# storj/uplink

Hardware: AMD Instinct MI355X
Metric: GiB/s erasure encode+decode (device-resident), RS(29,80) 64 MiB segments (higher is better)
Workload: dtype u8

## Files before the change

uplink_amd/csrc/ec_sets.cpp:

```cpp
#include "ec_internal.hpp"

namespace uplink_ec {
namespace capi {
namespace {


struct SetSeg {
    const uint8_t *in[kMaxOps];
    int num[kMaxOps];
    int missing[kMaxOps];
    int nin = 0, nstore = 0, rows = 0, nw = 2;
    uint8_t *out = nullptr;
};

int set_segment(const ec_ctx *c, int nshares, const int *nums, const uint8_t *const *pieces, uint8_t *out,
                bool decode, SetSeg &sg) {
    const int k = c->k;
    std::vector<int> order, ids;
    int rc = choose_shares(c, nshares, nums, order, ids);
    if (rc) return rc;
    if (decode)
        for (int i = 0; i < nshares; i++)
            if (nums[i] < 0 || nums[i] >= c->n) return EC_ERR_INVALID_SHARE;
    bool seen[256] = {};
// ... 32 lines not shown
    SetsSlot *sl = nullptr;
    const auto t_end = std::chrono::steady_clock::now() + std::chrono::milliseconds(SetsRing::kAcquireTimeoutMs);
    for (;;) {
        {
            std::lock_guard<std::mutex> g(R.mu);
            size_t live = 0;
            for (auto &x : R.slots) {
                live += !x->dead;
                if (!sl && x->idle()) sl = x.get();
            }
            if (!sl && live < SetsRing::kMaxSlots) {
                auto x = std::make_unique<SetsSlot>();
                if (hipHostMalloc((void **)&x->h_words, 4 * (SetsRing::kInitSegs + 1), kSetsHostFlags) != hipSuccess)
                    return nullptr;
                memset(x->h_words, 0, 4 * (SetsRing::kInitSegs + 1));
                x->words_cap = SetsRing::kInitSegs + 1;
                x->stage_cap = 0;
                R.slots.push_back(std::move(x));
                sl = R.slots.back().get();
            }
            if (sl) sl->busy = true;
        }
        if (sl) break;
        if (std::chrono::steady_clock::now() > t_end) return nullptr;
        std::this_thread::sleep_for(std::chrono::microseconds(20));
    }
    bool ok = true;
    if (sl->stage_cap < nseg) {
        size_t cap = std::max(sl->stage_cap ? 2 * sl->stage_cap : SetsRing::kInitSegs, (size_t)32);
        while (cap < nseg) cap *= 2;
        if (sl->h_stage) sl->old_host.push_back(sl->h_stage);
        for (void *p : {(void *)sl->d_stage, (void *)sl->d_desc, (void *)sl->d_words})
            if (p) sl->old_dev.push_back(p);
        sl->h_stage = nullptr, sl->d_stage = nullptr, sl->d_desc = nullptr, sl->d_words = nullptr;
        ok = hipHostMalloc((void **)&sl->h_stage, cap * sizeof(SetStage),
                           c->sets_stage_dma ? hipHostMallocDefault : kSetsHostFlags) == hipSuccess &&
             (!c->sets_stage_dma || hipMalloc(&sl->d_stage, cap * sizeof(SetStage)) == hipSuccess) &&
             hipMalloc(&sl->d_desc, cap * sizeof(SetDesc)) == hipSuccess &&
             hipMalloc(&sl->d_words, 4 * (cap + 1)) == hipSuccess;
        if (ok && cap + 1 > sl->words_cap) {
            uint32_t *hw = nullptr;
            ok = hipHostMalloc((void **)&hw, 4 * (cap + 1), kSetsHostFlags) == hipSuccess;
            if (ok) {
                hw[0] = sl->seq;
                sl->old_host.push_back(sl->h_words);
                sl->h_words = hw;
                sl->words_cap = cap + 1;
            }
        }
        sl->stage_cap = ok ? cap : 0;
    }
    if (ok && sl->tgt_cap < tgt_words) {
        size_t cap = std::max(sl->tgt_cap ? 2 * sl->tgt_cap : SetsRing::kInitTgtWords, (size_t)1);
        while (cap < tgt_words) cap *= 2;
        if (sl->d_tgt) sl->old_dev.push_back(sl->d_tgt);
        sl->d_tgt = nullptr;
        ok = hipMalloc(&sl->d_tgt, cap * 8) == hipSuccess;
        sl->tgt_cap = ok ? cap : 0;
    }
    if (!ok) {
        std::lock_guard<std::mutex> g(R.mu);
        sl->busy = false;
        return nullptr;
    }
    return sl;
}

void sets_release(ec_ctx *c, SetsSlot *sl) {
    std::lock_guard<std::mutex> g(c->sets.mu);
    sl->busy = false;
}

int sets_call(ec_ctx *c, std::vector<SetSeg> &segs, int64_t nstripes, hipStream_t s, std::vector<uint32_t> *bad) {
    const int k = c->k, ess = c->ess;
    const size_t nseg = segs.size();
    if (nseg == 0 || nstripes == 0) return EC_OK;
    if (c->sets_merge) {
        int nw = 2;
        for (auto &sg : segs) nw = std::max(nw, sg.nw);
        for (auto &sg : segs) sg.nw = nw;
    }
    {
        const int64_t tiles_seg = (nstripes * (ess / 16) + kTileChunksHost - 1) / kTileChunksHost;
        const int64_t per = share_max_tiles(4) / tiles_seg;
        if (per < 1) return EC_ERR_UNSUPPORTED;
        if ((int64_t)nseg > per) {
            for (size_t g0 = 0; g0 < nseg; g0 += (size_t)per) {
                std::vector<SetSeg> part(segs.begin() + g0, segs.begin() + std::min(nseg, g0 + (size_t)per));
                std::vector<uint32_t> pbad;
                const int rc = sets_call(c, part, nstripes, s, bad ? &pbad : nullptr);
                if (rc) return rc;
                if (bad) bad->insert(bad->end(), pbad.begin(), pbad.end());
            }
            return EC_OK;
        }
    }
    std::vector<int> idx(nseg);
    for (size_t g = 0; g < nseg; g++) idx[g] = (int)g;
    std::stable_sort(idx.begin(), idx.end(), [&](int x, int y) { return segs[x].nw < segs[y].nw; });
    std::vector<size_t> toff(nseg);
    size_t words = 0;
    for (size_t q = 0; q < nseg; q++) {
        toff[q] = words;
        words += (leaf_entries(segs[idx[q]].nin, segs[idx[q]].rows, segs[idx[q]].nw) + 7) & ~(size_t)7;
    }
    if (stream_is_capturing(s)) return EC_ERR_UNSUPPORTED;
    SetsSlot *sl = sets_acquire(c, nseg, words);
    if (!sl) return EC_ERR_DEVICE;
    SetStage one{};
    const bool in_args = nseg == 1 && !sl->d_stage;
    SetStage *stage = in_args ? &one : sl->h_stage;
    for (size_t q = 0; q < nseg; q++) {
        const SetSeg &sg = segs[idx[q]];
        SetStage &st = stage[q];
        SetDesc &d = st.d;
        for (int j = 0; j < sg.nin; j++) {
            d.in[j] = sg.in[j];
            d.copy_off[j] = j < k && sg.num[j] < k ? sg.num[j] * ess : -1;
            st.num[j] = sg.num[j];
        }
        for (int r = 0; r < sg.nstore; r++) {
            d.out_off[r] = sg.missing[r] * ess;
            st.missing[r] = sg.missing[r];
        }
        d.out = sg.out;
        d.tgt = sl->d_tgt + toff[q];
        d.zero_check = bad ? sl->d_words + 1 + q : nullptr;
        d.nin = sg.nin;
        d.nout = sg.rows;
        d.nstore = sg.nstore;
        d.status = 0;
        st.k = k;
        st.nw = sg.nw;
    }
    const uint32_t seq = sl->seq + 1;
    const int64_t chunks = nstripes * (ess / 16), tiles = (chunks + kTileChunksHost - 1) / kTileChunksHost;
    auto pass_args = [&](SetsArgs &a) {
        a.nstripes = nstripes;
        a.chunks_per_seg = chunks;
        a.tiles_per_seg = tiles;
        a.ess = ess;
        a.cps = ess / 16;
        a.k = k;
        a.done_ctr = sl->d_words;
        a.host_done = sl->h_words;
        a.seq = seq;
        a.total_wgs = (uint32_t)(tiles * (int64_t)nseg);
        a.chk_flag = c->d_chk;
        a.jt_base = c->jt_base;
    };
    hipError_t e = hipSuccess;
    if (in_args && !bad && c->sets_one && segs[0].nin <= kOneMaxIn && segs[0].nin * segs[0].rows <= kOneMaxCoef) {
        const SetSeg &sg = segs[0];
        SetOne p{};
        pass_args(p.a);
        p.a.total_tiles = tiles;
        for (int j = 0; j < sg.nin; j++) {
            p.in[j] = one.d.in[j];
            p.copy_off[j] = one.d.copy_off[j];
        }
        for (int r = 0; r < sg.nstore; r++) p.out_off[r] = one.d.out_off[r];
        p.out = sg.out;
        p.tgt = sl->d_tgt;
        p.nin = sg.nin;
        p.nout = sg.rows;
        p.nstore = sg.nstore;
        solve_rows(sg.num, k, sg.nin, sg.missing, sg.nstore, p.coef);
        e = launch_sets_one(p, sg.nw, s);
        if (e != hipSuccess) {
            sets_release(c, sl);
            return hip_fail(e);
        }
        sl->seq = seq;
        c->last_body = EC_BODY_JUMP_TABLE;
        const int rc = after_launch(c->d_chk, s);
        sets_release(c, sl);
        return rc;
    }
    if (sl->d_stage)
        e = hipMemcpyAsync(sl->d_stage, sl->h_stage, nseg * sizeof(SetStage), hipMemcpyHostToDevice, s);
    if (e == hipSuccess)
        e = in_args ? launch_sets_prep1(one, sl->d_desc, c->jt_base, sl->d_words, s)
                    : launch_sets_prep(sl->d_stage ? sl->d_stage : sl->h_stage, sl->d_desc, (int)nseg, c->jt_base,
                                       sl->d_words, s);
    if (e != hipSuccess) {
        sets_release(c, sl);
        return hip_fail(e);
    }
    for (size_t q0 = 0; q0 < nseg && e == hipSuccess;) {
        size_t q1 = q0;
        while (q1 < nseg && segs[idx[q1]].nw == segs[idx[q0]].nw) q1++;
        SetsArgs a{};
        pass_args(a);
        a.desc = sl->d_desc + q0;
        a.total_tiles = tiles * (int64_t)(q1 - q0);
        e = launch_matmul_sets(a, segs[idx[q0]].nw, s);
        q0 = q1;
    }
    if (e != hipSuccess) {
        const bool drained = hipStreamSynchronize(s) == hipSuccess && hipMemset(sl->d_words, 0, 4) == hipSuccess;
        std::lock_guard<std::mutex> g(c->sets.mu);
        sl->dead = !drained;
        sl->busy = false;
        return hip_fail(e);
    }
    sl->seq = seq;
    c->last_body = EC_BODY_JUMP_TABLE;
    int rc = after_launch(c->d_chk, s);
    if (bad && rc == EC_OK) {
        if (hipMemcpyAsync(sl->h_words + 1, sl->d_words + 1, 4 * nseg, hipMemcpyDeviceToHost, s) != hipSuccess ||
            hipStreamSynchronize(s) != hipSuccess)
            rc = EC_ERR_DEVICE;
        bad->assign(nseg, 0);
        for (size_t q = 0; q < nseg && rc == EC_OK; q++) (*bad)[idx[q]] = sl->h_words[1 + q];
    }
    sets_release(c, sl);
    return rc;
}


std::mutex g_builders_mu;
std::set<ec_ctx *> g_builders;

void sl_worker(ec_ctx *c) {
    (void)hipSetDevice(c->device);
    SlBuilder &B = c->slb;
    for (;;) {
        std::vector<int> ids;
        {
            std::unique_lock<std::mutex> g(B.mu);
            B.cv.wait(g, [&] { return B.stop || !B.q.empty(); });
            if (B.stop) break;
            ids = std::move(B.q.front());
            B.q.pop_front();
        }
        PlanPtr plan;
        if (get_plan(c, ids, &plan) == EC_OK && plan->rows >= 1 && plan->rows <= kMaxOps) ensure_sl(c, *plan);
        {
            std::lock_guard<std::mutex> g(B.mu);
            B.pending.erase(ids);
        }
        B.cv.notify_all();
    }
    std::lock_guard<std::mutex> g(B.mu);
    B.pending.clear();
    B.q.clear();
    B.cv.notify_all();
}

void stop_builders() {
    std::lock_guard<std::mutex> g(g_builders_mu);
    for (ec_ctx *c : g_builders) {
        {
            std::lock_guard<std::mutex> b(c->slb.mu);
            c->slb.stop = true;
        }
        c->slb.cv.notify_all();
        if (c->slb.th.joinable()) c->slb.th.join();
    }
    g_builders.clear();
}

void stop_builder_impl(ec_ctx *c) {
    {
        std::lock_guard<std::mutex> g(g_builders_mu);
        g_builders.erase(c);
        {
            std::lock_guard<std::mutex> b(c->slb.mu);
            c->slb.stop = true;
        }
        c->slb.cv.notify_all();
    }
    if (c->slb.th.joinable()) c->slb.th.join();
}

void sl_request(ec_ctx *c, const std::vector<int> &ids) {
    SlBuilder &B = c->slb;
    std::lock_guard<std::mutex> g(B.mu);
// ... 165 lines not shown
```

uplink_amd/csrc/rs_repair.hip:

```cpp
#include <hip/hip_runtime.h>

#include "gf256_field.hpp"
#include "rs_repair.hpp"
#include "rs_sets_tile.hpp"

namespace uplink_ec {
namespace {

using namespace dev;

__constant__ GfTables c_gf = make_gf_tables();

__global__ __launch_bounds__(256) void rs_repair_prep(const RepairStage *stage, RepairDesc *desc, uint64_t jt_base) {
    const RepairStage *st = stage + blockIdx.x;
    copy_desc(&st->d, desc + blockIdx.x);
    write_leaves(st->coef, st->entries, st->d.tgt, jt_base);
}

typedef const __attribute__((address_space(4))) RepairDesc ConstDesc;

struct RepairGeom {
    static constexpr bool kCopy = false, kOwnTable = false;
    const RepairArgs &a;
    ConstDesc *d;
    const int nstore;
    bool vA, vB;
    int64_t iA, iB, oA, oB;
    uint32_t bad = 0;

    __device__ __forceinline__ bool skip(int nin, int nout) const { return nin <= 0 || nout <= 0; }
    __device__ __forceinline__ void cols(int lane) {
        const int64_t tile = blockIdx.x;
        const int64_t seg = tile / a.tiles_per_seg;
        const int64_t qA = (tile - seg * a.tiles_per_seg) * kTileChunks + lane, qB = qA + 64;
        vA = qA < a.chunks_per_seg, vB = qB < a.chunks_per_seg;
        iA = vA ? qA * 16 : 0, iB = vB ? qB * 16 : 0;
        oA = qA * 16, oB = qB * 16;
    }
    __device__ __forceinline__ bool in_ok(const uint8_t *p, const uint8_t *share) const {
        return in_span(a, p, share, a.piece_len, 10);
    }
    __device__ __forceinline__ bool out_ok(const uint8_t *p, const uint8_t *row) const {
        return in_span(a, p, row, a.piece_len, 11);
    }
    __device__ __forceinline__ uint8_t *row_out(int r) const { return d->out[r]; }
    __device__ __forceinline__ int stored(int, int) const { return nstore; }
    __device__ __forceinline__ bool checks(int rbase, int cnt, int nst) const { return rbase + cnt > nst; }
    __device__ __forceinline__ void report(uint32_t any, int) { bad |= any; }
    __device__ __forceinline__ void finish(int lane) const {
        if (d->nout > nstore) {
            int32_t *st = d->status;
            if (__ballot(bad != 0) != 0 && lane == 0 && st) atomicOr(st, 1);
        }
    }
};

template <int NW>
__global__ __launch_bounds__(NW * 64, 4) void rs_repair(const RepairArgs a) {
    ConstDesc *d = (ConstDesc *)(a.desc + blockIdx.x / a.tiles_per_seg);
    RepairGeom G{a, d, d->nstore};
    share_tile<NW>(G);
}


__global__ __launch_bounds__(256) void rs_repair_sized_prep(const RepairSizedStage *stage, RepairSizedDesc *desc,
                                                            uint64_t jt_base) {
    const RepairSizedStage *st = stage + blockIdx.x;
    copy_desc(&st->d, desc + blockIdx.x);
    uint32_t *map = st->map;
    const int64_t ntiles = st->ntiles;
    for (int64_t i = threadIdx.x; i < ntiles; i += blockDim.x) map[i] = blockIdx.x;
    write_leaves(st->coef, st->entries, st->d.tgt, jt_base);
}

typedef const __attribute__((address_space(4))) RepairSizedDesc ConstSizedDesc;
typedef const __attribute__((address_space(4))) uint32_t ConstMap;

struct RepairSizedGeom {
    static constexpr bool kCopy = false, kOwnTable = false;
    const RepairSizedArgs &a;
    ConstSizedDesc *d;
    const int64_t tile;
    const int nstore;
    bool vA, vB;
    int64_t iA, iB, oA, oB;
    uint32_t bad = 0;

    __device__ __forceinline__ RepairSizedGeom(const RepairSizedArgs &a_, int64_t ctile)
        : a(a_),
          d((ConstSizedDesc *)(a_.desc + (uint32_t)__builtin_amdgcn_readfirstlane(((ConstMap *)a_.map)[ctile]))),
          tile(ctile - d->tile0), nstore(d->nstore) {}
    __device__ __forceinline__ bool skip(int nin, int nout) const { return nin <= 0 || nout <= 0 || tile < 0; }
    __device__ __forceinline__ void cols(int lane) {
        const int64_t chunks = d->chunks;
        const int64_t qA = tile * kTileChunks + lane, qB = qA + 64;
        vA = qA < chunks, vB = qB < chunks;
        iA = vA ? qA * 16 : 0, iB = vB ? qB * 16 : 0;
        oA = qA * 16, oB = qB * 16;
    }
    __device__ __forceinline__ bool in_ok(const uint8_t *p, const uint8_t *share) const {
        return in_span(a, p, share, d->piece_len, 14);
    }
    __device__ __forceinline__ bool out_ok(const uint8_t *p, const uint8_t *row) const {
        return in_span(a, p, row, d->piece_len, 15);
    }
    __device__ __forceinline__ uint8_t *row_out(int r) const { return d->out[r]; }
    __device__ __forceinline__ int stored(int, int) const { return nstore; }
    __device__ __forceinline__ bool checks(int rbase, int cnt, int nst) const { return rbase + cnt > nst; }
    __device__ __forceinline__ void report(uint32_t any, int) { bad |= any; }
    __device__ __forceinline__ void finish(int lane) const {
        if (d->nout > nstore) {
            int32_t *st = d->status;
            if (__ballot(bad != 0) != 0 && lane == 0 && st) atomicOr(st, 1);
        }
    }
};

template <int NW>
__global__ __launch_bounds__(NW * 64, 4) void rs_repair_sized(const RepairSizedArgs a) {
    RepairSizedGeom G(a, a.tile_base + blockIdx.x);
    share_tile<NW>(G);
}

__global__ __launch_bounds__(256) void rs_repair_check_bytes(const RsArgs a) {
    __shared__ uint8_t s_exp[512];
    __shared__ uint8_t s_log[256];
    __shared__ int s_bad;
    for (int i = threadIdx.x; i < 512; i += blockDim.x) s_exp[i] = c_gf.exp[i];
    for (int i = threadIdx.x; i < 256; i += blockDim.x) s_log[i] = c_gf.log[i];
    if (threadIdx.x == 0) s_bad = 0;
    __syncthreads();
    const int64_t cols = a.nstripes * a.ess;
    bool bad = false;
    for (int64_t col = (int64_t)blockIdx.x * blockDim.x + threadIdx.x; col < cols; col += (int64_t)gridDim.x * blockDim.x) {
        for (int r = 0; r < a.nout; r++) {
            uint8_t acc = 0;
            for (int j = 0; j < a.nin; j++) {
                const uint8_t x = a.in_base[a.in_off[j] + col];
                const uint8_t cv = a.coef[(int64_t)j * a.coef_ld + r];
                if (x && cv) acc ^= s_exp[s_log[x] + s_log[cv]];
            }
            bad = bad || acc != a.out_base[a.out_off[r] + col];
        }
    }
    if (bad) s_bad = 1;
    __syncthreads();
    if (threadIdx.x == 0 && s_bad) atomicOr(a.zero_check, 1u);
}

}

int repair_waves(int rows) { return rows <= 14 ? 2 : rows <= 24 ? 3 : rows <= 32 ? 4 : 8; }

hipError_t launch_repair_prep(const RepairStage *stage, RepairDesc *desc, int nseg, uint64_t jt_base, hipStream_t s) {
    if (nseg <= 0) return hipSuccess;
    hipLaunchKernelGGL(rs_repair_prep, dim3(nseg), dim3(256), 0, s, stage, desc, jt_base);
    return hipGetLastError();
}

hipError_t launch_repair(const RepairArgs &a, int nw, hipStream_t s) {
    return launch_share_tile(a, a.total_tiles, nw, s, rs_repair<2>, rs_repair<3>, rs_repair<4>, rs_repair<8>);
}
// ... 24 lines not shown
```

uplink_amd/csrc/rs_sets.hip:

```cpp
#include <hip/hip_runtime.h>

#include "../../include/uplink_ec.h"
#include "gf256_field.hpp"
#include "rs_device.hpp"
#include "rs_kernels.hpp"
#include "rs_sets.hpp"
#include "rs_sets_tile.hpp"

namespace uplink_ec {
namespace {

using namespace dev;

__constant__ GfTables c_gf = make_gf_tables();

__device__ __forceinline__ void solve_rows(const SetStage *st, uint64_t jt_base) {
    __shared__ uint8_t s_exp[512], s_log[256];
    __shared__ uint8_t s_x[kMaxOps];
    __shared__ uint8_t s_y[2 * kMaxOps];
    __shared__ int16_t s_lw[kMaxOps];
    __shared__ int16_t s_ln[2 * kMaxOps], s_hit[2 * kMaxOps];
    __shared__ int s_num[kMaxOps], s_miss[kMaxOps];
    __shared__ int s_acc[kMaxOps + 2 * kMaxOps];
    __shared__ int s_hdr[8];
// ... 4 lines not shown
        s_miss[i] = st->missing[i];
    }
    if (tid == 0) s_hdr[0] = st->d.nin;
    if (tid == 1) s_hdr[1] = st->d.nout;
    if (tid == 2) s_hdr[2] = st->d.nstore;
    if (tid == 3) s_hdr[3] = st->nw;
    if (tid == 4) s_hdr[4] = st->k;
    if (tid == 5) s_tgt = st->d.tgt;
    for (int i = tid; i < 512; i += nt) s_exp[i] = c_gf.exp[i];
    for (int i = tid; i < 256; i += nt) s_log[i] = c_gf.log[i];
    __syncthreads();
    const int nin = s_hdr[0], nout = s_hdr[1], nstore = s_hdr[2], nw = s_hdr[3], k = s_hdr[4];
    auto point = [&](int num) -> uint8_t { return num == 0 ? 0 : s_exp[(num - 1) % 255]; };
    for (int i = tid; i < k; i += nt) s_x[i] = point(s_num[i]);
    for (int i = tid; i < nout; i += nt) s_y[i] = point(i < nstore ? s_miss[i] : s_num[k + i - nstore]);
    for (int i = tid; i < k; i += nt) s_acc[i] = 0;
    for (int i = tid; i < nout; i += nt) {
        s_acc[kMaxOps + i] = 0;
        s_hit[i] = -1;
    }
    __syncthreads();
    for (int e = tid; e < (k + nout) * k; e += nt) {
        const int a = e / k, t = e - a * k;
        if (a < k) {
            if (t != a) atomicAdd(&s_acc[a], (int)s_log[s_x[a] ^ s_x[t]]);
        } else {
            const uint8_t d = s_y[a - k] ^ s_x[t];
            if (d) atomicAdd(&s_acc[kMaxOps + a - k], (int)s_log[d]);
            else s_hit[a - k] = (int16_t)t;
        }
    }
    __syncthreads();
    for (int i = tid; i < k; i += nt) s_lw[i] = (int16_t)(s_acc[i] % 255);
    for (int i = tid; i < nout; i += nt) s_ln[i] = (int16_t)(s_acc[kMaxOps + i] % 255);
    __syncthreads();
    const int npass = npass_of(nout, nw), per_pass = nin * nw * kRows;
    uint64_t *tgt = s_tgt;
    for (int e = tid; e < npass * per_pass; e += nt) {
        const int pass = e / per_pass, rem = e - pass * per_pass;
        const int j = rem / (nw * kRows), g = (rem / kRows) % nw, o = rem % kRows;
        int rb, cn;
        rows_of(pass, npass, nout, nw, g, rb, cn);
        const int oo = o - (kRows - cn);
        uint32_t c = 0;
        if (oo >= 0) {
            const int r = rb + oo;
            if (j >= k) {
                c = (uint32_t)(r >= nstore && j - k == r - nstore);
            } else if (s_hit[r] >= 0) {
                c = (uint32_t)(s_hit[r] == j);
            } else {
                const int l = s_ln[r] - s_log[s_y[r] ^ s_x[j]] - s_lw[j];
                c = s_exp[((l % 255) + 255) % 255];
            }
        }
        tgt[e] = jt_base + (uint64_t)c * RS_JT_SLOT;
    }
}

__device__ __forceinline__ void prep_one(const SetStage *st, SetDesc *dd, uint64_t jt_base, uint32_t *done_ctr) {
    const int tid = threadIdx.x;
    copy_desc(&st->d, dd);
    if (tid == 6) {
        uint32_t *zc = st->d.zero_check;
        if (zc) *zc = 0u;
    }
    if (tid == 7 && blockIdx.x == 0 && done_ctr) *done_ctr = 0u;
    solve_rows(st, jt_base);
}

__global__ __launch_bounds__(256) void rs_sets_prep(const SetStage *stage, SetDesc *desc, uint64_t jt_base,
                                                    uint32_t *done_ctr) {
    prep_one(stage + blockIdx.x, desc + blockIdx.x, jt_base, done_ctr);
}

__global__ __launch_bounds__(256) void rs_sets_prep1(const SetStage stage, SetDesc *desc, uint64_t jt_base,
                                                     uint32_t *done_ctr) {
    prep_one(&stage, desc, jt_base, done_ctr);
}

typedef const __attribute__((address_space(4))) SetDesc ConstDesc;
typedef const __attribute__((address_space(4))) SetOne ConstOne;

template <class D>
struct SetsGeom : StripeGeom<D> {
    static constexpr bool kOwnTable = __is_same(D, ConstOne);
    using StripeGeom<D>::d;
    const SetsArgs &a;

    __device__ __forceinline__ SetsGeom(const SetsArgs &a_, D *d_) : StripeGeom<D>{d_}, a(a_) {}
    __device__ __forceinline__ bool skip(int nin, int) const { return !(d->status == 0 && nin > 0); }
    __device__ __forceinline__ void cols(int lane) {
        const int64_t tile = blockIdx.x;
        const int64_t seg = kOwnTable ? 0 : tile / a.tiles_per_seg;
        this->stripe_cols((tile - seg * a.tiles_per_seg) * kTileChunks + lane, a.chunks_per_seg, a.cps, a.ess, a.k);
    }
    __device__ __forceinline__ bool in_ok(const uint8_t *p, const uint8_t *share) const {
        return in_span(a, p, share, a.nstripes * a.ess, 8);
    }
    __device__ __forceinline__ bool out_ok(const uint8_t *p, const uint8_t *) const {
        return in_span(a, p, this->out, a.nstripes * a.ess * a.k, 9);
    }
    template <int NW>
    __device__ __forceinline__ void write_table(int npass, int nin, int nout) const {
        uint64_t *t = d->tgt;
        for (int e = threadIdx.x; e < npass * nin * NW * kRows; e += NW * 64) {
            const int pass = e / (nin * NW * kRows), rem = e - pass * (nin * NW * kRows);
            const int j = rem / (NW * kRows), g = (rem / kRows) % NW, o = rem % kRows;
            int rb, cn;
            rows_of(pass, npass, nout, NW, g, rb, cn);
            const int oo = o - (kRows - cn);
            const uint32_t c = oo >= 0 ? d->coef[(rb + oo) * nin + j] : 0u;
            t[e] = a.jt_base + (uint64_t)c * RS_JT_SLOT;
        }
    }
};

__device__ __forceinline__ void sets_done(const SetsArgs &a) {
    if (a.done_ctr) {
        lds_barrier();
        if (threadIdx.x == 0) {
            const uint32_t old = atomicAdd(a.done_ctr, 1u);
            if (old + 1 == a.total_wgs) {
                atomicExch(a.done_ctr, 0u);
                __hip_atomic_store(a.host_done, a.seq, __ATOMIC_RELEASE, __HIP_MEMORY_SCOPE_SYSTEM);
            }
        }
    }
}

template <int NW>
__global__ __launch_bounds__(NW * 64, 4) void rs_matmul_sets(const SetsArgs a) {
    SetsGeom<ConstDesc> G{a, (ConstDesc *)(a.desc + blockIdx.x / a.tiles_per_seg)};
    share_tile<NW>(G);
    sets_done(a);
}

template <int NW>
__global__ __launch_bounds__(NW * 64, 4) void rs_sets_one(const SetOne p) {
    SetsGeom<ConstOne> G{p.a, (ConstOne *)&p};
    share_tile<NW>(G);
    sets_done(p.a);
}

}

int sets_waves(int rows) { return rows <= 14 ? 2 : rows <= 24 ? 3 : 4; }

hipError_t launch_sets_prep(const SetStage *stage, SetDesc *desc, int nseg, uint64_t jt_base, uint32_t *done_ctr,
                            hipStream_t s) {
    if (nseg <= 0) return hipSuccess;
    hipLaunchKernelGGL(rs_sets_prep, dim3(nseg), dim3(256), 0, s, stage, desc, jt_base, done_ctr);
    return hipGetLastError();
}

hipError_t launch_sets_prep1(const SetStage &stage, SetDesc *desc, uint64_t jt_base, uint32_t *done_ctr,
                             hipStream_t s) {
    hipLaunchKernelGGL(rs_sets_prep1, dim3(1), dim3(256), 0, s, stage, desc, jt_base, done_ctr);
    return hipGetLastError();
}

hipError_t launch_sets_one(const SetOne &p, int nw, hipStream_t s) {
    if (p.a.total_tiles <= 0) return hipSuccess;
    if (p.nin > kOneMaxIn || p.nin * p.nout > kOneMaxCoef) return hipErrorInvalidValue;
    return launch_share_tile(p, p.a.total_tiles, nw, s, rs_sets_one<2>, rs_sets_one<3>, rs_sets_one<4>);
}

hipError_t launch_matmul_sets(const SetsArgs &a, int nw, hipStream_t s) {
    return launch_share_tile(a, a.total_tiles, nw, s, rs_matmul_sets<2>, rs_matmul_sets<3>, rs_matmul_sets<4>);
}

}
```

uplink_amd/csrc/rs_sets.hpp:

```cpp
#pragma once
#include "rs_args.hpp"
#include "rs_rows.hpp"

namespace uplink_ec {

struct SetDesc {
    const uint8_t *in[kMaxOps];
    uint8_t *out;
    uint64_t *tgt;
    uint32_t *zero_check;
    int32_t nin, nout, nstore, status;
    int32_t copy_off[kMaxOps];
    int32_t out_off[kMaxOps];
};
static_assert(sizeof(SetDesc) % 8 == 0, "copied as 8-byte words");

struct SetStage {
    SetDesc d;
    int32_t num[kMaxOps];
    int32_t missing[kMaxOps];
    int32_t k, nw, pad0, pad1;
};

struct SetsArgs {
    const SetDesc *desc;
    int64_t nstripes, chunks_per_seg, tiles_per_seg, total_tiles;
    int32_t ess, cps, k, pad;
    uint32_t *done_ctr;
    uint32_t *host_done;
    uint32_t seq, total_wgs;
    uint32_t *chk_flag;
    uint64_t jt_base;
};

constexpr int64_t kTileChunksHost = 128;

int sets_waves(int rows);
hipError_t launch_sets_prep(const SetStage *stage, SetDesc *desc, int nseg, uint64_t jt_base, uint32_t *done_ctr,
                            hipStream_t s);
hipError_t launch_sets_prep1(const SetStage &stage, SetDesc *desc, uint64_t jt_base, uint32_t *done_ctr,
                             hipStream_t s);
static_assert(sizeof(SetStage) + 3 * sizeof(void *) <= 4096, "a launch's arguments are at most 4 KB");
hipError_t launch_matmul_sets(const SetsArgs &a, int nw, hipStream_t s);

constexpr int kOneMaxIn = 64, kOneMaxCoef = 2048;
struct SetOne {
    SetsArgs a;
    const uint8_t *in[kOneMaxIn];
    uint8_t *out;
    uint64_t *tgt;
    uint32_t *zero_check;
    int32_t nin, nout, nstore, status;
    int32_t copy_off[kOneMaxIn];
    int32_t out_off[kOneMaxIn];
    uint8_t coef[kOneMaxCoef];
};
static_assert(sizeof(SetOne) <= 4096, "a launch's arguments are at most 4 KB");
hipError_t launch_sets_one(const SetOne &p, int nw, hipStream_t s);
hipError_t jt_table_base_addr(uint64_t *out, hipStream_t s);

}
```

uplink_amd/csrc/rs_sets_tile.hpp:

```cpp
#pragma once
#include <hip/hip_runtime.h>

#include "rs_device.hpp"
#include "rs_rows.hpp"

namespace uplink_ec {
namespace dev {

template <class Args>
__device__ __forceinline__ bool in_span(const Args &a, const uint8_t *p, const uint8_t *lo, int64_t len, int site) {
#ifdef UPLINK_EC_CHECKED
    if (p >= lo && p + 16 <= lo + len) return true;
    if (a.chk_flag) atomicCAS(a.chk_flag, 0u, (uint32_t)site);
    return false;
#else
    (void)a, (void)p, (void)lo, (void)len, (void)site;
    return true;
#endif
}

template <class Desc>
__device__ __forceinline__ void copy_desc(const Desc *src, Desc *dst) {
    static_assert(sizeof(Desc) % 8 == 0, "copied as 8-byte words");
    const uint64_t *s = (const uint64_t *)src;
    uint64_t *d = (uint64_t *)dst;
    for (int i = threadIdx.x; i < (int)(sizeof(Desc) / 8); i += blockDim.x) d[i] = s[i];
}

__device__ __forceinline__ void write_leaves(const uint8_t *coef, int64_t entries, uint64_t *tgt, uint64_t jt_base) {
    const uint4 *cf = (const uint4 *)coef;
    const int64_t n16 = entries / 16;
    for (int64_t i = threadIdx.x; i < n16; i += blockDim.x) {
        const uint4 v = cf[i];
        const uint32_t w[4] = {v.x, v.y, v.z, v.w};
#pragma unroll
        for (int b = 0; b < 16; b++)
            tgt[i * 16 + b] = jt_base + (uint64_t)((w[b >> 2] >> (8 * (b & 3))) & 0xFFu) * RS_JT_SLOT;
    }
}

template <class D>
struct StripeGeom {
    static constexpr bool kCopy = true;
    D *d;
    bool vA, vB;
    int64_t iA, iB, oA, oB;
    uint8_t *out;
    uint32_t *zc;

    __device__ __forceinline__ void stripe_cols(int64_t qA, int64_t chunks, int cps_, int ess, int k) {
        const int64_t qB = qA + 64;
        vA = qA < chunks, vB = qB < chunks;
        const uint32_t cps = (uint32_t)cps_;
        const uint32_t sA = (uint32_t)qA / cps, tA = (uint32_t)qA - sA * cps;
        const uint32_t sB = (uint32_t)qB / cps, tB = (uint32_t)qB - sB * cps;
        iA = vA ? (int64_t)sA * ess + tA * 16 : 0, iB = vB ? (int64_t)sB * ess + tB * 16 : 0;
        oA = (int64_t)sA * k * ess + tA * 16, oB = (int64_t)sB * k * ess + tB * 16;
        out = d->out;
    }
    __device__ __forceinline__ int copy_off(int j) const { return d->copy_off[j]; }
    __device__ __forceinline__ uint8_t *out_base() const { return out; }
    __device__ __forceinline__ uint8_t *row_out(int r) const { return out + d->out_off[r]; }
    __device__ __forceinline__ int stored(int rbase, int cnt) {
        zc = d->zero_check;
        return zc ? d->nstore : rbase + cnt;
    }
    __device__ __forceinline__ bool checks(int, int, int) const { return zc != nullptr; }
    __device__ __forceinline__ void report(uint32_t any, int lane) const {
        if (__ballot(any != 0) != 0 && lane == 0) atomicAdd(zc, 1u);
    }
    __device__ __forceinline__ void finish(int) const {}
};

template <int NW, class Geom>
__device__ __forceinline__ void share_tile(Geom &G) {
    constexpr int JC = 2 * NW, PER = 2, OPW = kRows, SLOT = JC * 2048;
    extern __shared__ __attribute__((aligned(16))) uint32_t smem[];
    u32x4 *ring = (u32x4 *)smem;
    const int lane = threadIdx.x & 63;
    const int wave = __builtin_amdgcn_readfirstlane(threadIdx.x >> 6);
    const int group = (wave + (int)(blockIdx.x % NW)) % NW;
    const uint32_t ring_addr = (uint32_t)(uintptr_t)smem;
    const int nin = G.d->nin, nout = G.d->nout;
    if (G.skip(nin, nout)) return;
    G.cols(lane);
    const bool vA = G.vA, vB = G.vB;
    const int nchunks = (nin + JC - 1) / JC;
    const int CH = (nin + nchunks - 1) / nchunks;
    const int npass = npass_of(nout, NW);
    auto owned = [&](int ch) -> int {
        const int jn = nin - ch * CH < CH ? nin - ch * CH : CH;
        return wave < jn ? (jn - wave + NW - 1) / NW : 0;
    };
    auto issue = [&](int ch) {
        const uint32_t d0 = ring_addr + (uint32_t)((ch & 1) * SLOT);
#pragma unroll
        for (int i = 0; i < PER; i++) {
            const int j = wave + NW * i;
            if (i < owned(ch)) {
                const uint8_t *p = G.d->in[ch * CH + j];
                const uint8_t *pa = p + G.iA, *pb = p + G.iB;
                if (!G.in_ok(pa, p)) pa = p;
                if (!G.in_ok(pb, p)) pb = p;
                const uint32_t dst = __builtin_amdgcn_readfirstlane(d0 + (uint32_t)(j * 2048));
                dma_1k(pa, dst);
                dma_1k(pb, dst + 1024);
            }
        }
    };
    if constexpr (Geom::kOwnTable) {
        issue(0);
        G.template write_table<NW>(npass, nin, nout);
    }
    for (int pass = 0; pass < npass; pass++) {
        int rbase, cnt;
        rows_of(pass, npass, nout, NW, group, rbase, cnt);
        if (!Geom::kOwnTable || pass > 0) issue(0);
        u32x8 acc[OPW];
#pragma unroll
        for (int o = 0; o < OPW; o++) acc[o] = (u32x8){0, 0, 0, 0, 0, 0, 0, 0};
        for (int ch = 0; ch < nchunks; ch++) {
            wait_vm(0);
            const int j0 = ch * CH;
            u32x4 *slot = ring + (ch & 1) * (SLOT / 16);
#pragma unroll
            for (int i = 0; i < PER; i++) {
                const int j = wave + NW * i;
                if (i < owned(ch)) {
                    const u32x4 A4 = slot[j * 128 + lane], B4 = slot[j * 128 + 64 + lane];
                    if constexpr (Geom::kCopy) {
                        const int co = G.copy_off(j0 + j);
                        if (pass == 0 && co >= 0) {
                            uint8_t *p = G.out_base() + co;
                            if (vA && G.out_ok(p + G.oA, p)) st16<true>(p + G.oA, A4.x, A4.y, A4.z, A4.w);
                            if (vB && G.out_ok(p + G.oB, p)) st16<true>(p + G.oB, B4.x, B4.y, B4.z, B4.w);
                        }
                    }
                    uint32_t w[8] = {A4.x, A4.y, A4.z, A4.w, B4.x, B4.y, B4.z, B4.w};
                    bitslice8(w);
                    slot[j * 128 + lane] = (u32x4){w[0], w[1], w[2], w[3]};
                    slot[j * 128 + 64 + lane] = (u32x4){w[4], w[5], w[6], w[7]};
                }
            }
            lds_barrier();
            if (ch + 1 < nchunks) issue(ch + 1);
            if (cnt > 0) {
                const int jn = nin - j0 < CH ? nin - j0 : CH;
                jt_inputs(acc, ring_addr + (uint32_t)((ch & 1) * SLOT) + (uint32_t)lane * 16,
                          G.d->tgt + ((int64_t)(pass * nin + j0) * NW + group) * OPW, (uint32_t)(NW * OPW * 8),
                          (uint32_t)(OPW - cnt), (uint32_t)jn);
            }
        }
        uint32_t rows[OPW][8];
#pragma unroll
        for (int o = 0; o < OPW; o++)
#pragma unroll
            for (int p = 0; p < 8; p++) rows[o][p] = acc[o][p];
        const int nst = G.stored(rbase, cnt);
        if (G.checks(rbase, cnt, nst)) {
            uint32_t any = 0;
#pragma unroll
            for (int o = 0; o < OPW; o++)
                if (o < cnt && rbase + o >= nst)
#pragma unroll
                    for (int p = 0; p < 8; p++) any |= rows[o][p];
            any &= (vA ? 0x0F0F0F0Fu : 0u) | (vB ? 0xF0F0F0F0u : 0u);
            G.report(any, lane);
        }
        static_for<OPW>([&]<int O>() {
            if (O < cnt && rbase + O < nst) {
                uint32_t w[8];
#pragma unroll
                for (int p = 0; p < 8; p++) w[p] = rows[O][p];
                unbitslice8(w);
                uint8_t *p = G.row_out(rbase + O);
                if (vA && G.out_ok(p + G.oA, p)) st16<true>(p + G.oA, w[0], w[1], w[2], w[3]);
                if (vB && G.out_ok(p + G.oB, p)) st16<true>(p + G.oB, w[4], w[5], w[6], w[7]);
            }
        });
        lds_barrier();
    }
    G.finish(lane);
}

template <class Args>
inline hipError_t launch_share_tile(const Args &a, int64_t tiles, int nw, hipStream_t s, void (*k2)(Args),
                                    void (*k3)(Args), void (*k4)(Args), void (*k8)(Args) = nullptr) {
    if (tiles <= 0) return hipSuccess;
    if (tiles > share_max_tiles(nw)) return hipErrorInvalidValue;
    void (*const k)(Args) = nw == 2 ? k2 : nw == 3 ? k3 : nw == 4 ? k4 : nw == 8 ? k8 : nullptr;
    if (!k) return hipErrorInvalidValue;
    hipLaunchKernelGGL(k, dim3((unsigned)tiles), dim3(nw * 64), (size_t)2 * 2 * nw * 2048, s, a);
    return hipGetLastError();
}

}
}
```

uplink_amd/csrc/rs_sized.hip:

```cpp
#include <hip/hip_runtime.h>

#include "rs_sets_tile.hpp"
#include "rs_sized.hpp"

namespace uplink_ec {
namespace {

using namespace dev;

__global__ __launch_bounds__(256) void rs_sized_prep(const SizedStage *stage, SizedDesc *desc, uint64_t jt_base) {
    const SizedStage *st = stage + blockIdx.x;
    const int tid = threadIdx.x;
    copy_desc(&st->d, desc + blockIdx.x);
    if (tid == 0) {
        uint32_t *zc = st->d.zero_check;
        if (zc) *zc = 0u;
    }
    uint32_t *map = st->map;
    const int64_t ntiles = st->ntiles;
    for (int64_t i = tid; i < ntiles; i += blockDim.x) map[i] = blockIdx.x;
    write_leaves(st->coef, st->entries, st->d.tgt, jt_base);
}

typedef const __attribute__((address_space(4))) SizedDesc ConstDesc;
typedef const __attribute__((address_space(4))) uint32_t ConstMap;

struct SizedGeom : StripeGeom<ConstDesc> {
    static constexpr bool kOwnTable = false;
    const SizedArgs &a;
    const int64_t tile;

    __device__ __forceinline__ SizedGeom(const SizedArgs &a_, int64_t ctile)
        : StripeGeom<ConstDesc>{(ConstDesc *)(a_.desc +
                                              (uint32_t)__builtin_amdgcn_readfirstlane(((ConstMap *)a_.map)[ctile]))},
          a(a_), tile(ctile - d->tile0) {}
    __device__ __forceinline__ bool skip(int nin, int) const { return nin <= 0 || tile < 0; }
    __device__ __forceinline__ void cols(int lane) { stripe_cols(tile * kTileChunks + lane, d->chunks, a.cps, a.ess, a.k); }
    __device__ __forceinline__ bool in_ok(const uint8_t *p, const uint8_t *share) const {
        return in_span(a, p, share, d->piece_len, 12);
    }
    __device__ __forceinline__ bool out_ok(const uint8_t *p, const uint8_t *) const {
        return in_span(a, p, out, d->spad, 13);
    }
};

template <int NW>
__global__ __launch_bounds__(NW * 64, 4) void rs_matmul_sized(const SizedArgs a) {
    SizedGeom G(a, a.tile_base + blockIdx.x);
    share_tile<NW>(G);
}

}

hipError_t launch_sized_prep(const SizedStage *stage, SizedDesc *desc, int nseg, uint64_t jt_base, hipStream_t s) {
    if (nseg <= 0) return hipSuccess;
    hipLaunchKernelGGL(rs_sized_prep, dim3(nseg), dim3(256), 0, s, stage, desc, jt_base);
    return hipGetLastError();
}

hipError_t launch_matmul_sized(const SizedArgs &a, int nw, hipStream_t s) {
    return launch_share_tile(a, a.total_tiles, nw, s, rs_matmul_sized<2>, rs_matmul_sized<3>, rs_matmul_sized<4>);
}

}
```

Baseline: 837.1.

## Process multiple tiles per workgroup with cross-tile load pipelining and early done counting

Each sets workgroup now handles a group of four consecutive tiles instead of one. The LDS double-buffer ring runs continuously across chunk, pass and tile boundaries, so the next tile's input loads are issued while the current tile is still computing. Waits on outstanding stores are counted per row instead of draining all vector memory. Completion counting moves into the geometry and happens before the final stores. The aim is to cut launch/workgroup overhead and load-latency bubbles, at the cost of fewer workgroups (less parallelism for small segments) and more complex index bookkeeping.

```diff
diff --git a/uplink_amd/csrc/ec_sets.cpp b/uplink_amd/csrc/ec_sets.cpp
--- a/uplink_amd/csrc/ec_sets.cpp
+++ b/uplink_amd/csrc/ec_sets.cpp
@@ -138,7 +138,7 @@
     }
     {
         const int64_t tiles_seg = (nstripes * (ess / 16) + kTileChunksHost - 1) / kTileChunksHost;
-        const int64_t per = share_max_tiles(4) / tiles_seg;
+        const int64_t per = share_max_tiles(4) / sets_groups(tiles_seg);
         if (per < 1) return EC_ERR_UNSUPPORTED;
         if ((int64_t)nseg > per) {
             for (size_t g0 = 0; g0 < nseg; g0 += (size_t)per) {
@@ -191,6 +191,7 @@
     }
     const uint32_t seq = sl->seq + 1;
     const int64_t chunks = nstripes * (ess / 16), tiles = (chunks + kTileChunksHost - 1) / kTileChunksHost;
+    const int64_t groups = sets_groups(tiles);
     auto pass_args = [&](SetsArgs &a) {
         a.nstripes = nstripes;
         a.chunks_per_seg = chunks;
@@ -201,7 +202,7 @@
         a.done_ctr = sl->d_words;
         a.host_done = sl->h_words;
         a.seq = seq;
-        a.total_wgs = (uint32_t)(tiles * (int64_t)nseg);
+        a.total_wgs = (uint32_t)(groups * (int64_t)nseg);
         a.chk_flag = c->d_chk;
         a.jt_base = c->jt_base;
     };
@@ -210,7 +211,7 @@
         const SetSeg &sg = segs[0];
         SetOne p{};
         pass_args(p.a);
-        p.a.total_tiles = tiles;
+        p.a.launch_wgs = groups;
         for (int j = 0; j < sg.nin; j++) {
             p.in[j] = one.d.in[j];
             p.copy_off[j] = one.d.copy_off[j];
@@ -249,7 +250,7 @@
         SetsArgs a{};
         pass_args(a);
         a.desc = sl->d_desc + q0;
-        a.total_tiles = tiles * (int64_t)(q1 - q0);
+        a.launch_wgs = groups * (int64_t)(q1 - q0);
         e = launch_matmul_sets(a, segs[idx[q0]].nw, s);
         q0 = q1;
     }
diff --git a/uplink_amd/csrc/rs_repair.hip b/uplink_amd/csrc/rs_repair.hip
--- a/uplink_amd/csrc/rs_repair.hip
+++ b/uplink_amd/csrc/rs_repair.hip
@@ -21,6 +21,7 @@
 
 struct RepairGeom {
     static constexpr bool kCopy = false, kOwnTable = false;
+    static constexpr int kTilesPerGroup = 1;
     const RepairArgs &a;
     ConstDesc *d;
     const int nstore;
@@ -78,6 +79,7 @@
 
 struct RepairSizedGeom {
     static constexpr bool kCopy = false, kOwnTable = false;
+    static constexpr int kTilesPerGroup = 1;
     const RepairSizedArgs &a;
     ConstSizedDesc *d;
     const int64_t tile;
diff --git a/uplink_amd/csrc/rs_sets.hip b/uplink_amd/csrc/rs_sets.hip
--- a/uplink_amd/csrc/rs_sets.hip
+++ b/uplink_amd/csrc/rs_sets.hip
@@ -110,18 +110,60 @@
 typedef const __attribute__((address_space(4))) SetDesc ConstDesc;
 typedef const __attribute__((address_space(4))) SetOne ConstOne;
 
+#ifndef UPLINK_SETS_DONE
+#define UPLINK_SETS_DONE 2
+#endif
+
 template <class D>
 struct SetsGeom : StripeGeom<D> {
     static constexpr bool kOwnTable = __is_same(D, ConstOne);
+    static constexpr int kTilesPerGroup = kSetsTilesPerGroup;
     using StripeGeom<D>::d;
     const SetsArgs &a;
+    int ntl, left;
+    int64_t in0;
+    uint32_t sA, tA, sB, tB;
+    uint32_t old;
+    bool early = false;
 
     __device__ __forceinline__ SetsGeom(const SetsArgs &a_, D *d_) : StripeGeom<D>{d_}, a(a_) {}
     __device__ __forceinline__ bool skip(int nin, int) const { return !(d->status == 0 && nin > 0); }
     __device__ __forceinline__ void cols(int lane) {
-        const int64_t tile = blockIdx.x;
-        const int64_t seg = kOwnTable ? 0 : tile / a.tiles_per_seg;
-        this->stripe_cols((tile - seg * a.tiles_per_seg) * kTileChunks + lane, a.chunks_per_seg, a.cps, a.ess, a.k);
+        const uint32_t gps = (uint32_t)sets_groups(a.tiles_per_seg);
+        const uint32_t grp = kOwnTable ? blockIdx.x : blockIdx.x % gps;
+        const int64_t tile0 = (int64_t)grp * kTilesPerGroup;
+        const int64_t qA = tile0 * kTileChunks + lane;
+        if constexpr (kTilesPerGroup == 1) {
+            this->stripe_cols(qA, a.chunks_per_seg, a.cps, a.ess, a.k);
+        } else {
+            const int64_t more = a.chunks_per_seg - tile0 * kTileChunks;
+            ntl = (int)(a.tiles_per_seg - tile0 < kTilesPerGroup ? a.tiles_per_seg - tile0 : kTilesPerGroup);
+            left = (int)(more < kTilesPerGroup * kTileChunks ? more : kTilesPerGroup * kTileChunks);
+            in0 = tile0 * kTileChunks * 16;
+            const uint32_t cps = (uint32_t)a.cps;
+            sA = (uint32_t)qA / cps, tA = (uint32_t)qA - sA * cps;
+            sB = (uint32_t)(qA + 64) / cps, tB = (uint32_t)(qA + 64) - sB * cps;
+            this->vA = lane < left, this->vB = lane + 64 < left;
+            this->out = d->out;
+        }
+    }
+    __device__ __forceinline__ int tiles() const { return ntl; }
+    __device__ __forceinline__ bool full() const { return left >= kTileChunks; }
+    __device__ __forceinline__ int64_t in_A(int lane, bool next) const {
+        const int q = lane + (next ? kTileChunks : 0);
+        return q < left ? in0 + q * 16 : 0;
+    }
+    __device__ __forceinline__ int64_t in_B(int lane, bool next) const { return in_A(lane + 64, next); }
+    __device__ __forceinline__ int64_t out_A() const { return (int64_t)((uint64_t)sA * (uint32_t)(a.k * a.ess)) + tA * 16; }
+    __device__ __forceinline__ int64_t out_B() const { return (int64_t)((uint64_t)sB * (uint32_t)(a.k * a.ess)) + tB * 16; }
+    __device__ __forceinline__ void next_tile(int lane) {
+        const uint32_t cps = (uint32_t)a.cps, dq = (uint32_t)kTileChunks / cps, dr = (uint32_t)kTileChunks - dq * cps;
+        const bool cA = tA + dr >= cps, cB = tB + dr >= cps;
+        tA = tA + dr - (cA ? cps : 0u), sA += dq + (cA ? 1u : 0u);
+        tB = tB + dr - (cB ? cps : 0u), sB += dq + (cB ? 1u : 0u);
+        in0 += kTileChunks * 16;
+        left -= kTileChunks;
+        this->vA = lane < left, this->vB = lane + 64 < left;
     }
     __device__ __forceinline__ bool in_ok(const uint8_t *p, const uint8_t *share) const {
         return in_span(a, p, share, a.nstripes * a.ess, 8);
@@ -142,33 +184,42 @@
             t[e] = a.jt_base + (uint64_t)c * RS_JT_SLOT;
         }
     }
+    __device__ __forceinline__ void count() {
+        lds_barrier();
+        if (threadIdx.x == 0) old = atomicAdd(a.done_ctr, 1u);
+    }
+    __device__ __forceinline__ void counted() const {
+        if (threadIdx.x == 0 && old + 1 == a.total_wgs) {
+            atomicExch(a.done_ctr, 0u);
+            __hip_atomic_store(a.host_done, a.seq, __ATOMIC_RELEASE, __HIP_MEMORY_SCOPE_SYSTEM);
+        }
+    }
+    static constexpr bool kDoneEarly = UPLINK_SETS_DONE == 2;
+    __device__ __forceinline__ void done_begin() {
+        if (a.done_ctr) {
+            asm volatile("" : "+s"(this->out), "+s"(this->zc));
+            count();
+            early = true;
+        }
+    }
+    __device__ __forceinline__ void done_end() {
+        if (UPLINK_SETS_DONE != 0 && a.done_ctr) {
+            if (!early) count();
+            counted();
+        }
+    }
 };
-
-__device__ __forceinline__ void sets_done(const SetsArgs &a) {
-    if (a.done_ctr) {
-        lds_barrier();
-        if (threadIdx.x == 0) {
-            const uint32_t old = atomicAdd(a.done_ctr, 1u);
-            if (old + 1 == a.total_wgs) {
-                atomicExch(a.done_ctr, 0u);
-                __hip_atomic_store(a.host_done, a.seq, __ATOMIC_RELEASE, __HIP_MEMORY_SCOPE_SYSTEM);
-            }
-        }
-    }
-}
 
 template <int NW>
 __global__ __launch_bounds__(NW * 64, 4) void rs_matmul_sets(const SetsArgs a) {
-    SetsGeom<ConstDesc> G{a, (ConstDesc *)(a.desc + blockIdx.x / a.tiles_per_seg)};
+    SetsGeom<ConstDesc> G{a, (ConstDesc *)(a.desc + blockIdx.x / (uint32_t)sets_groups(a.tiles_per_seg))};
     share_tile<NW>(G);
-    sets_done(a);
 }
 
 template <int NW>
 __global__ __launch_bounds__(NW * 64, 4) void rs_sets_one(const SetOne p) {
     SetsGeom<ConstOne> G{p.a, (ConstOne *)&p};
     share_tile<NW>(G);
-    sets_done(p.a);
 }
 
 }
@@ -189,13 +240,13 @@
 }
 
 hipError_t launch_sets_one(const SetOne &p, int nw, hipStream_t s) {
-    if (p.a.total_tiles <= 0) return hipSuccess;
+    if (p.a.launch_wgs <= 0) return hipSuccess;
     if (p.nin > kOneMaxIn || p.nin * p.nout > kOneMaxCoef) return hipErrorInvalidValue;
-    return launch_share_tile(p, p.a.total_tiles, nw, s, rs_sets_one<2>, rs_sets_one<3>, rs_sets_one<4>);
+    return launch_share_tile(p, p.a.launch_wgs, nw, s, rs_sets_one<2>, rs_sets_one<3>, rs_sets_one<4>);
 }
 
 hipError_t launch_matmul_sets(const SetsArgs &a, int nw, hipStream_t s) {
-    return launch_share_tile(a, a.total_tiles, nw, s, rs_matmul_sets<2>, rs_matmul_sets<3>, rs_matmul_sets<4>);
-}
-
-}
+    return launch_share_tile(a, a.launch_wgs, nw, s, rs_matmul_sets<2>, rs_matmul_sets<3>, rs_matmul_sets<4>);
+}
+
+}
diff --git a/uplink_amd/csrc/rs_sets.hpp b/uplink_amd/csrc/rs_sets.hpp
--- a/uplink_amd/csrc/rs_sets.hpp
+++ b/uplink_amd/csrc/rs_sets.hpp
@@ -24,7 +24,7 @@
 
 struct SetsArgs {
     const SetDesc *desc;
-    int64_t nstripes, chunks_per_seg, tiles_per_seg, total_tiles;
+    int64_t nstripes, chunks_per_seg, tiles_per_seg, launch_wgs;
     int32_t ess, cps, k, pad;
     uint32_t *done_ctr;
     uint32_t *host_done;
@@ -34,6 +34,13 @@
 };
 
 constexpr int64_t kTileChunksHost = 128;
+
+#ifndef UPLINK_SETS_TILES
+#define UPLINK_SETS_TILES 4
+#endif
+constexpr int kSetsTilesPerGroup = UPLINK_SETS_TILES;
+static_assert(kSetsTilesPerGroup >= 1 && (kSetsTilesPerGroup & (kSetsTilesPerGroup - 1)) == 0, "a power of two");
+constexpr int64_t sets_groups(int64_t tiles) { return (tiles + kSetsTilesPerGroup - 1) / kSetsTilesPerGroup; }
 
 int sets_waves(int rows);
 hipError_t launch_sets_prep(const SetStage *stage, SetDesc *desc, int nseg, uint64_t jt_base, uint32_t *done_ctr,
diff --git a/uplink_amd/csrc/rs_sets_tile.hpp b/uplink_amd/csrc/rs_sets_tile.hpp
--- a/uplink_amd/csrc/rs_sets_tile.hpp
+++ b/uplink_amd/csrc/rs_sets_tile.hpp
@@ -3,6 +3,10 @@
 
 #include "rs_device.hpp"
 #include "rs_rows.hpp"
+
+#ifndef UPLINK_SETS_PIPELINE
+#define UPLINK_SETS_PIPELINE 1
+#endif
 
 namespace uplink_ec {
 namespace dev {
@@ -72,9 +76,38 @@
     __device__ __forceinline__ void finish(int) const {}
 };
 
+template <class Geom>
+constexpr bool done_early() {
+    if constexpr (requires { Geom::kDoneEarly; }) return Geom::kDoneEarly;
+    else return false;
+}
+
+__device__ __forceinline__ void wait_vm_rows(int rows) {
+    static_assert(kRows == 8);
+    switch (rows) {
+        case 1: wait_vm(2); break;
+        case 2: wait_vm(4); break;
+        case 3: wait_vm(6); break;
+        case 4: wait_vm(8); break;
+        case 5: wait_vm(10); break;
+        case 6: wait_vm(12); break;
+        case 7: wait_vm(14); break;
+        case 8: wait_vm(16); break;
+        default: wait_vm(0);
+    }
+}
+
 template <int NW, class Geom>
 __device__ __forceinline__ void share_tile(Geom &G) {
     constexpr int JC = 2 * NW, PER = 2, OPW = kRows, SLOT = JC * 2048;
+    constexpr bool kRun = Geom::kTilesPerGroup > 1 && UPLINK_SETS_PIPELINE;
+    constexpr bool kDone = requires { G.done_end(); };
+    constexpr bool kEarly = done_early<Geom>();
+#ifdef UPLINK_EC_CHECKED
+    constexpr bool kCountStores = false;
+#else
+    constexpr bool kCountStores = true;
+#endif
     extern __shared__ __attribute__((aligned(16))) uint32_t smem[];
     u32x4 *ring = (u32x4 *)smem;
     const int lane = threadIdx.x & 63;
@@ -82,9 +115,13 @@
     const int group = (wave + (int)(blockIdx.x % NW)) % NW;
     const uint32_t ring_addr = (uint32_t)(uintptr_t)smem;
     const int nin = G.d->nin, nout = G.d->nout;
-    if (G.skip(nin, nout)) return;
+    if (G.skip(nin, nout)) {
+        if constexpr (kDone) G.done_end();
+        return;
+    }
     G.cols(lane);
-    const bool vA = G.vA, vB = G.vB;
+    int ntl = 1;
+    if constexpr (Geom::kTilesPerGroup > 1) ntl = G.tiles();
     const int nchunks = (nin + JC - 1) / JC;
     const int CH = (nin + nchunks - 1) / nchunks;
     const int npass = npass_of(nout, NW);
@@ -92,14 +129,14 @@
         const int jn = nin - ch * CH < CH ? nin - ch * CH : CH;
         return wave < jn ? (jn - wave + NW - 1) / NW : 0;
     };
-    auto issue = [&](int ch) {
-        const uint32_t d0 = ring_addr + (uint32_t)((ch & 1) * SLOT);
+    auto issue = [&](int ch, int sb, int64_t iA, int64_t iB) {
+        const uint32_t d0 = ring_addr + (uint32_t)(sb * SLOT);
 #pragma unroll
         for (int i = 0; i < PER; i++) {
             const int j = wave + NW * i;
             if (i < owned(ch)) {
                 const uint8_t *p = G.d->in[ch * CH + j];
-                const uint8_t *pa = p + G.iA, *pb = p + G.iB;
+                const uint8_t *pa = p + iA, *pb = p + iB;
                 if (!G.in_ok(pa, p)) pa = p;
                 if (!G.in_ok(pb, p)) pb = p;
                 const uint32_t dst = __builtin_amdgcn_readfirstlane(d0 + (uint32_t)(j * 2048));
@@ -108,79 +145,134 @@
             }
         }
     };
-    if constexpr (Geom::kOwnTable) {
-        issue(0);
-        G.template write_table<NW>(npass, nin, nout);
-    }
-    for (int pass = 0; pass < npass; pass++) {
-        int rbase, cnt;
-        rows_of(pass, npass, nout, NW, group, rbase, cnt);
-        if (!Geom::kOwnTable || pass > 0) issue(0);
-        u32x8 acc[OPW];
-#pragma unroll
-        for (int o = 0; o < OPW; o++) acc[o] = (u32x8){0, 0, 0, 0, 0, 0, 0, 0};
-        for (int ch = 0; ch < nchunks; ch++) {
-            wait_vm(0);
-            const int j0 = ch * CH;
-            u32x4 *slot = ring + (ch & 1) * (SLOT / 16);
-#pragma unroll
-            for (int i = 0; i < PER; i++) {
-                const int j = wave + NW * i;
-                if (i < owned(ch)) {
-                    const u32x4 A4 = slot[j * 128 + lane], B4 = slot[j * 128 + 64 + lane];
-                    if constexpr (Geom::kCopy) {
-                        const int co = G.copy_off(j0 + j);
-                        if (pass == 0 && co >= 0) {
-                            uint8_t *p = G.out_base() + co;
-                            if (vA && G.out_ok(p + G.oA, p)) st16<true>(p + G.oA, A4.x, A4.y, A4.z, A4.w);
-                            if (vB && G.out_ok(p + G.oB, p)) st16<true>(p + G.oB, B4.x, B4.y, B4.z, B4.w);
+    auto in_A = [&](bool next) -> int64_t {
+        if constexpr (Geom::kTilesPerGroup > 1) return G.in_A(lane, next);
+        else return G.iA;
+    };
+    auto in_B = [&](bool next) -> int64_t {
+        if constexpr (Geom::kTilesPerGroup > 1) return G.in_B(lane, next);
+        else return G.iB;
+    };
+    auto out_A = [&]() -> int64_t {
+        if constexpr (Geom::kTilesPerGroup > 1) return G.out_A();
+        else return G.oA;
+    };
+    auto out_B = [&]() -> int64_t {
+        if constexpr (Geom::kTilesPerGroup > 1) return G.out_B();
+        else return G.oB;
+    };
+    if constexpr (Geom::kOwnTable || kRun) issue(0, 0, in_A(false), in_B(false));
+    if constexpr (Geom::kOwnTable) G.template write_table<NW>(npass, nin, nout);
+    int run = 0;
+    int after = 0;
+    for (int tl = ntl; tl > 0; tl--) {
+        const bool vA = G.vA, vB = G.vB;
+        for (int pass = 0; pass < npass; pass++) {
+            int rbase, cnt;
+            rows_of(pass, npass, nout, NW, group, rbase, cnt);
+            if constexpr (!kRun)
+                if (!Geom::kOwnTable || pass > 0 || tl < ntl) issue(0, 0, in_A(false), in_B(false));
+            u32x8 acc[OPW];
+#pragma unroll
+            for (int o = 0; o < OPW; o++) acc[o] = (u32x8){0, 0, 0, 0, 0, 0, 0, 0};
+            for (int ch = 0; ch < nchunks; ch++) {
+                const int sb = kRun ? run : ch & 1;
+                if constexpr (kRun) {
+                    wait_vm_rows(after);
+                    after = 0;
+                } else {
+                    wait_vm(0);
+                }
+                const int j0 = ch * CH;
+                u32x4 *slot = ring + sb * (SLOT / 16);
+#pragma unroll
+                for (int i = 0; i < PER; i++) {
+                    const int j = wave + NW * i;
+                    if (i < owned(ch)) {
+                        const u32x4 A4 = slot[j * 128 + lane], B4 = slot[j * 128 + 64 + lane];
+                        if constexpr (Geom::kCopy) {
+                            const int co = G.copy_off(j0 + j);
+                            if (pass == 0 && co >= 0) {
+                                uint8_t *p = G.out_base() + co;
+                                const int64_t oA = out_A(), oB = out_B();
+                                if (vA && G.out_ok(p + oA, p)) st16<true>(p + oA, A4.x, A4.y, A4.z, A4.w);
+                                if (vB && G.out_ok(p + oB, p)) st16<true>(p + oB, B4.x, B4.y, B4.z, B4.w);
+                            }
                         }
+                        uint32_t w[8] = {A4.x, A4.y, A4.z, A4.w, B4.x, B4.y, B4.z, B4.w};
+                        bitslice8(w);
+                        slot[j * 128 + lane] = (u32x4){w[0], w[1], w[2], w[3]};
+                        slot[j * 128 + 64 + lane] = (u32x4){w[4], w[5], w[6], w[7]};
                     }
-                    uint32_t w[8] = {A4.x, A4.y, A4.z, A4.w, B4.x, B4.y, B4.z, B4.w};
-                    bitslice8(w);
-                    slot[j * 128 + lane] = (u32x4){w[0], w[1], w[2], w[3]};
-                    slot[j * 128 + 64 + lane] = (u32x4){w[4], w[5], w[6], w[7]};
-                }
-            }
-            lds_barrier();
-            if (ch + 1 < nchunks) issue(ch + 1);
-            if (cnt > 0) {
-                const int jn = nin - j0 < CH ? nin - j0 : CH;
-                jt_inputs(acc, ring_addr + (uint32_t)((ch & 1) * SLOT) + (uint32_t)lane * 16,
-                          G.d->tgt + ((int64_t)(pass * nin + j0) * NW + group) * OPW, (uint32_t)(NW * OPW * 8),
-                          (uint32_t)(OPW - cnt), (uint32_t)jn);
+                }
+                lds_barrier();
+                if constexpr (kRun) {
+                    const bool wrap = ch + 1 == nchunks, step = wrap && pass + 1 == npass;
+                    if (!step || tl > 1) issue(wrap ? 0 : ch + 1, sb ^ 1, in_A(step), in_B(step));
+                } else if (ch + 1 < nchunks) {
+                    issue(ch + 1, sb ^ 1, in_A(false), in_B(false));
+                }
+                if (cnt > 0) {
+                    const int jn = nin - j0 < CH ? nin - j0 : CH;
+                    jt_inputs(acc, ring_addr + (uint32_t)(sb * SLOT) + (uint32_t)lane * 16,
+                              G.d->tgt + ((int64_t)(pass * nin + j0) * NW + group) * OPW, (uint32_t)(NW * OPW * 8),
+                              (uint32_t)(OPW - cnt), (uint32_t)jn);
+                }
+                if constexpr (kRun) run ^= 1;
+            }
+            uint32_t rows[OPW][8];
+#pragma unroll
+            for (int o = 0; o < OPW; o++)
+#pragma unroll
+                for (int p = 0; p < 8; p++) rows[o][p] = acc[o][p];
+            const int nst = G.stored(rbase, cnt);
+            uint8_t *rp[OPW];
+            if constexpr (kEarly) {
+#pragma unroll
+                for (int o = 0; o < OPW; o++) {
+                    rp[o] = o < cnt && rbase + o < nst ? G.row_out(rbase + o) : nullptr;
+                    asm volatile("" : "+s"(rp[o]));
+                }
+                if (pass + 1 == npass && tl == 1) G.done_begin();
+            }
+            if (G.checks(rbase, cnt, nst)) {
+                uint32_t any = 0;
+#pragma unroll
+                for (int o = 0; o < OPW; o++)
+                    if (o < cnt && rbase + o >= nst)
+#pragma unroll
+                        for (int p = 0; p < 8; p++) any |= rows[o][p];
+                any &= (vA ? 0x0F0F0F0Fu : 0u) | (vB ? 0xF0F0F0F0u : 0u);
+                G.report(any, lane);
+            }
+            static_for<OPW>([&]<int O>() {
+                if (O < cnt && rbase + O < nst) {
+                    uint32_t w[8];
+#pragma unroll
+                    for (int p = 0; p < 8; p++) w[p] = rows[O][p];
+                    unbitslice8(w);
+                    uint8_t *p;
+                    if constexpr (kEarly) p = rp[O];
+                    else p = G.row_out(rbase + O);
+                    const int64_t oA = out_A(), oB = out_B();
+                    if (vA && G.out_ok(p + oA, p)) st16<true>(p + oA, w[0], w[1], w[2], w[3]);
+                    if (vB && G.out_ok(p + oB, p)) st16<true>(p + oB, w[4], w[5], w[6], w[7]);
+                }
+            });
+            if constexpr (kRun) {
+                if constexpr (kCountStores) {
+                    const int ns = nst - rbase < cnt ? nst - rbase : cnt;
+                    after = G.full() && ns > 0 ? ns : 0;
+                }
+            } else {
+                lds_barrier();
             }
         }
-        uint32_t rows[OPW][8];
-#pragma unroll
-        for (int o = 0; o < OPW; o++)
-#pragma unroll
-            for (int p = 0; p < 8; p++) rows[o][p] = acc[o][p];
-        const int nst = G.stored(rbase, cnt);
-        if (G.checks(rbase, cnt, nst)) {
-            uint32_t any = 0;
-#pragma unroll
-            for (int o = 0; o < OPW; o++)
-                if (o < cnt && rbase + o >= nst)
-#pragma unroll
-                    for (int p = 0; p < 8; p++) any |= rows[o][p];
-            any &= (vA ? 0x0F0F0F0Fu : 0u) | (vB ? 0xF0F0F0F0u : 0u);
-            G.report(any, lane);
-        }
-        static_for<OPW>([&]<int O>() {
-            if (O < cnt && rbase + O < nst) {
-                uint32_t w[8];
-#pragma unroll
-                for (int p = 0; p < 8; p++) w[p] = rows[O][p];
-                unbitslice8(w);
-                uint8_t *p = G.row_out(rbase + O);
-                if (vA && G.out_ok(p + G.oA, p)) st16<true>(p + G.oA, w[0], w[1], w[2], w[3]);
-                if (vB && G.out_ok(p + G.oB, p)) st16<true>(p + G.oB, w[4], w[5], w[6], w[7]);
-            }
-        });
-        lds_barrier();
+        if constexpr (Geom::kTilesPerGroup > 1)
+            if (tl > 1) G.next_tile(lane);
     }
     G.finish(lane);
+    if constexpr (kDone) G.done_end();
 }
 
 template <class Args>
diff --git a/uplink_amd/csrc/rs_sized.hip b/uplink_amd/csrc/rs_sized.hip
--- a/uplink_amd/csrc/rs_sized.hip
+++ b/uplink_amd/csrc/rs_sized.hip
@@ -27,6 +27,7 @@
 
 struct SizedGeom : StripeGeom<ConstDesc> {
     static constexpr bool kOwnTable = false;
+    static constexpr int kTilesPerGroup = 1;
     const SizedArgs &a;
     const int64_t tile;
 
```

Result: slower. 826.8 (-1.2%).
